# Gepetto/mpc-interface

Measured on AMD Instinct MI355X. Metric: QP assemblies/sec (P,q,G,h), biped N=16 batched, higher is better.
Workload: dtype f64; 1 GPU; C2 biped LIPM N=16 no=36 nc=76, per-instance (A,B)/given/aim, K1 on chip; batch_per_gpu=4096, global_batch=4096, streams=2

## Files before the change

include/mpcasm.h:

```cpp
#ifndef MPCASM_H
#define MPCASM_H

#include <stddef.h>
#include <stdint.h>

#ifdef __cplusplus
extern "C" {
#endif

typedef enum mpcasm_status {
  MPCASM_OK = 0,
  MPCASM_ERR_ARG = -1,
  MPCASM_ERR_PLAN = -2,
  MPCASM_ERR_HIP = -3,
  MPCASM_ERR_NODEVICE = -4,
  MPCASM_ERR_LIMIT = -5
} mpcasm_status;

typedef struct mpcasm_plan mpcasm_plan;


int mpcasm_abi_version(void);
int mpcasm_device_count(void);
int mpcasm_last_hip(void);
const char* mpcasm_status_string(int status);
enum { MPCASM_OPT_PATH = 1, MPCASM_OPT_PHASE_MASK = 2, MPCASM_OPT_RESIDENT_PER_CU = 3, MPCASM_OPT_JIT = 4,
       MPCASM_OPT_P_DIRECT = 5, MPCASM_OPT_RESIDENT_GRID = 6, MPCASM_OPT_JIT_FETCH_RUNS = 7 };
int mpcasm_set_option(int option, int value);
int mpcasm_plan_set_option(mpcasm_plan* plan, int option, int value);
int mpcasm_resident_lds_bytes(const int32_t* h_itab, size_t n_itab, const double* h_dtab, size_t n_dtab,
                              int64_t out[2]);
int mpcasm_jit_check(const int32_t* h_itab, size_t n_itab, const double* h_dtab, size_t n_dtab,
                     char* log, size_t log_capacity);
int mpcasm_fetch_segments(const int32_t* h_itab, size_t n_itab, const double* h_dtab, size_t n_dtab,
                          int limit, int32_t* out, size_t capacity, int64_t* n_words);

int mpcasm_plan_prepare(const mpcasm_plan* plan, int batch);
int mpcasm_jit_stats(int64_t out[3]);

int mpcasm_fill_su(const double* d_A, const double* d_B, double* d_S, double* d_U,
                   int batch, int N, int n, int m, int ltv, void* stream);

int mpcasm_plan_create(const int32_t* h_itab, size_t n_itab,
                       const double* h_dtab, size_t n_dtab,
                       mpcasm_plan** out_plan);
int mpcasm_plan_destroy(mpcasm_plan* plan);

int mpcasm_plan_sizes(const mpcasm_plan* plan, int64_t out[8]);

int mpcasm_plan_csc_sizes(const mpcasm_plan* plan, int64_t out[2]);
// ... 105 lines not shown
```

mpc-interface_amd/csrc/capi.hip:

```cpp
#include <hip/hip_runtime.h>
#include <stdint.h>
#include <stdlib.h>
#include <string.h>

#include <algorithm>
#include <cmath>
#include <mutex>
#include <new>
#include <string>
#include <vector>

#include "jit.h"
#include "kernels.h"

using namespace mpcasm;

namespace mpcasm {
int g_p_direct = 0;
extern int g_path;
extern int g_phase_mask;
extern int g_resident_per_cu, g_resident_grid;
}

struct mpcasm_plan {
// ... 1052 lines not shown
    g_phase_mask = value;
    return MPCASM_OK;
  }
  if (option == MPCASM_OPT_P_DIRECT) {
    if (value < 0 || value > 2) return MPCASM_ERR_ARG;
    g_p_direct = value;
    return MPCASM_OK;
  }
  if (option == MPCASM_OPT_JIT) {
    if (value < 0 || value > 2) return MPCASM_ERR_ARG;
    g_jit = value;
    return MPCASM_OK;
  }
  if (option == MPCASM_OPT_RESIDENT_PER_CU) {
    if (value < 0 || value > 16) return MPCASM_ERR_ARG;
    g_resident_per_cu = value;
    return MPCASM_OK;
  }
  if (option == MPCASM_OPT_JIT_FETCH_RUNS) {
    if (value < 0 || value > FS_MAX) return MPCASM_ERR_ARG;
    g_jit_fetch_runs = value;
    return MPCASM_OK;
  }
  if (option == MPCASM_OPT_RESIDENT_GRID) {
    if (value < 0 || value > (1 << 20)) return MPCASM_ERR_ARG;
    g_resident_grid = value;
    return MPCASM_OK;
  }
  return MPCASM_ERR_ARG;
}

int mpcasm_plan_set_option(mpcasm_plan* plan, int option, int value) {
  if (!plan) return MPCASM_ERR_ARG;
  if (option == MPCASM_OPT_PATH && value >= -1 && value <= 4) plan->opt_path = value;
  else if (option == MPCASM_OPT_JIT && value >= -1 && value <= 2) plan->opt_jit = value;
  else if (option == MPCASM_OPT_RESIDENT_PER_CU && value >= -1 && value <= 16) plan->opt_per_cu = value;
  else if (option == MPCASM_OPT_RESIDENT_GRID && value >= -1 && value <= (1 << 20)) plan->opt_grid = value;
  else return MPCASM_ERR_ARG;
  return MPCASM_OK;
}

const char* mpcasm_status_string(int status) {
  switch (status) {
    case MPCASM_OK: return "ok";
    case MPCASM_ERR_ARG: return "invalid argument";
    case MPCASM_ERR_PLAN: return "malformed plan tables";
// ... 76 lines not shown
  const int rc = validate_plan(h_itab, h_dtab, n_itab, n_dtab);
  if (rc != MPCASM_OK) return rc;
  PlanDev d;
  memset(&d, 0, sizeof d);
  plan_dev_from_tables(h_itab, &d);
  for (int direct = 0; direct < 2; ++direct) {
    d.rs_p_direct = 1 - direct;
    out[direct] = (int64_t)resident_lds_bytes(d);
  }
  return MPCASM_OK;
}

int mpcasm_jit_check(const int32_t* h_itab, size_t n_itab, const double* h_dtab, size_t n_dtab,
                     char* log, size_t log_capacity) {
  if (!h_itab || (n_dtab && !h_dtab)) return MPCASM_ERR_ARG;
  if (log && log_capacity) log[0] = 0;
  const int rc = validate_plan(h_itab, h_dtab, n_itab, n_dtab);
  if (rc != MPCASM_OK) return rc;
  PlanDev d;
  memset(&d, 0, sizeof d);
  plan_dev_from_tables(h_itab, &d);
  if (!d.rs_ok) return MPCASM_ERR_LIMIT;
  std::vector<char> code;
  std::string text;
  const int small = resident_p_direct_for(d, 1), large = resident_p_direct_for(d, 1 << 30);
  int out = MPCASM_OK;
  if (!jit_available()) {
    text = "libhiprtc.so could not be loaded";
    out = MPCASM_ERR_LIMIT;
  } else {
    for (int form : {small, large}) {
      if (form == large && small != large && out != MPCASM_OK) break;
      d.rs_p_direct = form;
      out = jit_code_for(jit_spec_header(d, h_itab, g_jit_fetch_runs), false, 0xBF, &code, &text) ? MPCASM_OK : MPCASM_ERR_HIP;
      if (small == large) break;
    }
  }
  if (log && log_capacity) {
    strncpy(log, text.c_str(), log_capacity - 1);
    log[log_capacity - 1] = 0;
  }
  return out;
}

int mpcasm_fetch_segments(const int32_t* h_itab, size_t n_itab, const double* h_dtab, size_t n_dtab,
                          int limit, int32_t* out, size_t capacity, int64_t* n_words) {
  if (!h_itab || (n_dtab && !h_dtab) || !n_words || (capacity && !out) || limit < 0) return MPCASM_ERR_ARG;
  const int rc = validate_plan(h_itab, h_dtab, n_itab, n_dtab);
  if (rc != MPCASM_OK) return rc;
  PlanDev d;
  memset(&d, 0, sizeof d);
  plan_dev_from_tables(h_itab, &d);
  if (!d.rs_ok) return MPCASM_ERR_LIMIT;
  const std::vector<int32_t> words = jit_fetch_plan(d, h_itab, limit);
  *n_words = (int64_t)words.size();
  if (words.size() > capacity) return MPCASM_ERR_LIMIT;
  if (!words.empty()) memcpy(out, words.data(), words.size() * sizeof(int32_t));
  return MPCASM_OK;
}
// ... 496 lines not shown
```

mpc-interface_amd/csrc/device_prims.h:

```cpp
#pragma once
#ifndef __HIPCC_RTC__
#include <hip/hip_runtime.h>
#include <stdint.h>
#endif

namespace mpcasm {

typedef double f64x4 __attribute__((ext_vector_type(4)));

__device__ __forceinline__ f64x4 mfma_f64_16x16x4(double a, double b, f64x4 c) {
  return __builtin_amdgcn_mfma_f64_16x16x4f64(a, b, c, 0, 0, 0);
}
__device__ __forceinline__ double mfma_f64_4x4x4(double a, double b, double c) {
  return __builtin_amdgcn_mfma_f64_4x4x4f64(a, b, c, 0, 0, 0);
}

template <int OA, int OB, int RB>
__device__ __forceinline__ double mfma_trip16(unsigned pa, unsigned pb, double sum) {
  static_assert(OA >= 0 && OB >= 0 && OA + 3 * RB < 65536 && OB + 3 * RB < 65536, "ds_read offset field");
  double a0, a1, a2, a3, b0, b1, b2, b3;
  asm volatile(
      "ds_read_b64 %1, %9 offset:%11\n\t"
      "ds_read_b64 %5, %10 offset:%15\n\t"
      "ds_read_b64 %2, %9 offset:%12\n\t"
      "ds_read_b64 %6, %10 offset:%16\n\t"
      "ds_read_b64 %3, %9 offset:%13\n\t"
      "ds_read_b64 %7, %10 offset:%17\n\t"
      "ds_read_b64 %4, %9 offset:%14\n\t"
      "ds_read_b64 %8, %10 offset:%18\n\t"
      "s_waitcnt lgkmcnt(6)\n\t"
      "v_mfma_f64_4x4x4_4b_f64 %0, %1, %5, %0\n\t"
      "s_waitcnt lgkmcnt(4)\n\t"
      "s_nop 2\n\t"
      "v_mfma_f64_4x4x4_4b_f64 %0, %2, %6, %0\n\t"
      "s_waitcnt lgkmcnt(2)\n\t"
      "s_nop 2\n\t"
      "v_mfma_f64_4x4x4_4b_f64 %0, %3, %7, %0\n\t"
      "s_waitcnt lgkmcnt(0)\n\t"
      "s_nop 2\n\t"
      "v_mfma_f64_4x4x4_4b_f64 %0, %4, %8, %0\n\t"
      "s_nop 5"
      : "+v"(sum), "=&v"(a0), "=&v"(a1), "=&v"(a2), "=&v"(a3), "=&v"(b0), "=&v"(b1), "=&v"(b2), "=&v"(b3)
      : "v"(pa), "v"(pb), "n"(OA), "n"(OA + RB), "n"(OA + 2 * RB), "n"(OA + 3 * RB), "n"(OB),
        "n"(OB + RB), "n"(OB + 2 * RB), "n"(OB + 3 * RB));
  return sum;
}

__device__ __forceinline__ double mfma_trip16_at(unsigned pa, unsigned pb, unsigned row_bytes, double sum) {
  double a0, a1, a2, a3, b0, b1, b2, b3;
  const unsigned pa1 = pa + row_bytes, pa2 = pa1 + row_bytes, pa3 = pa2 + row_bytes;
  const unsigned pb1 = pb + row_bytes, pb2 = pb1 + row_bytes, pb3 = pb2 + row_bytes;
  asm volatile(
      "ds_read_b64 %1, %9\n\t"
      "ds_read_b64 %5, %13\n\t"
      "ds_read_b64 %2, %10\n\t"
      "ds_read_b64 %6, %14\n\t"
      "ds_read_b64 %3, %11\n\t"
      "ds_read_b64 %7, %15\n\t"
      "ds_read_b64 %4, %12\n\t"
      "ds_read_b64 %8, %16\n\t"
      "s_waitcnt lgkmcnt(6)\n\t"
      "v_mfma_f64_4x4x4_4b_f64 %0, %1, %5, %0\n\t"
      "s_waitcnt lgkmcnt(4)\n\t"
      "s_nop 2\n\t"
      "v_mfma_f64_4x4x4_4b_f64 %0, %2, %6, %0\n\t"
      "s_waitcnt lgkmcnt(2)\n\t"
      "s_nop 2\n\t"
      "v_mfma_f64_4x4x4_4b_f64 %0, %3, %7, %0\n\t"
      "s_waitcnt lgkmcnt(0)\n\t"
// ... 41 lines not shown
```

mpc-interface_amd/csrc/jit.h:

```cpp
#pragma once
#include <hip/hip_runtime.h>
#include <stdint.h>

#include <string>
#include <vector>

#include "plan_dev.h"

namespace mpcasm {

extern int g_jit;
extern int g_jit_fetch_runs;
extern int g_phase_mask;

std::string jit_spec_header(const PlanDev& d, const int32_t* h_itab, int seg_limit = FS_MAX);
std::vector<int32_t> jit_fetch_plan(const PlanDev& d, const int32_t* h_itab, int seg_limit);
int jit_compile(const std::string& header, std::vector<char>* code, std::string* log,
                bool stamps = false, int phases = 0xBF);
const void* jit_kernel_for(const PlanDev& d, const int32_t* h_itab, int device, int batch,
                           size_t lds_bytes);
bool jit_code_for(const std::string& header, bool stamps, int phases, std::vector<char>* code,
                  std::string* log, bool distrust_disk = false);
bool jit_available();
void jit_stats(long out[3]);
void jit_forget(const void* itab);
int jit_launch(const void* kernel, const PlanDev& p, const SrcTable& src, const double* params,
               const double* given, double* P, double* q, double* G, double* h, int batch,
               int num_cus, int per_cu_limit, int grid_limit, void* work, hipStream_t stream, hipError_t* err);

}
```

mpc-interface_amd/csrc/jit.hip:

```cpp
#include <dlfcn.h>
#include <hip/hip_runtime.h>
#include <stdint.h>
#include <stdio.h>
#include <stdlib.h>
#include <string.h>

#include <sys/stat.h>
#include <sys/types.h>
#include <unistd.h>

#include <atomic>
#include <condition_variable>
#include <iterator>
#include <map>
#include <mutex>
#include <string>
#include <vector>

#include "jit.h"
#include "kernels.h"

namespace mpcasm {

int g_jit = 0;
int g_jit_fetch_runs = FS_MAX;

namespace {

#include "jit_embed.inc"

constexpr int JIT_MIN_BATCH = 512;

struct Rtc {
  typedef struct _hiprtcProgram* Program;
  int (*create)(Program*, const char*, const char*, int, const char* const*, const char* const*);
  int (*compile)(Program, int, const char* const*);
  int (*log_size)(Program, size_t*);
  int (*get_log)(Program, char*);
  int (*code_size)(Program, size_t*);
  int (*get_code)(Program, char*);
  int (*destroy)(Program*);
  bool ok = false;
};

const Rtc& rtc() {
  static Rtc r;
  static std::once_flag once;
  std::call_once(once, [] {
// ... 101 lines not shown
        for (int w = 0; w < FS_WORDS; ++w) append(table, w ? ", %lld" : "%lld", g < n ? fetch[at + 3 + g * FS_WORDS + w] : 0);
        table += "}, ";
      }
      table += "},\n";
    }
    if (chunks == 0) counts = "0", table = "  {},\n";
    s += std::string("constexpr int FSEG_") + name + "_N[] = {" + counts + "};\n";
    s += std::string("constexpr int FSEG_") + name + "[][8][6] = {\n" + table + "};\n";
    s += std::string("constexpr unsigned FSEG_") + name + "_TABLE = ";
    append(s, "%lldu;\n", on_table);
  }
  s += "constexpr int LTI[4][8] = {\n";
  for (int g = 0; g < RS_LTI_MAX; ++g) {
    s += "  {";
    for (int w = 0; w < RS_LTI_WORDS; ++w)
      append(s, w ? ", %lld" : "%lld", g < d.rs_nlti ? it[d.off_rs_lti + g * RS_LTI_WORDS + w] : 0);
    s += "},\n";
  }
  s += "};\n}  // namespace spec\n}  // namespace mpcasm\n";
  return s;
}

int jit_compile(const std::string& header, std::vector<char>* code, std::string* log, bool stamps,
                int phases) {
  const Rtc& r = rtc();
  if (!r.ok) {
    if (log) *log = "libhiprtc.so could not be loaded";
    return MPCASM_ERR_LIMIT;
  }
  const char* headers[] = {header.c_str(), k_src_device_prims, k_src_plan_dev, k_src_plan_tables};
  const char* names[] = {"plan_spec.h", "device_prims.h", "plan_dev.h", "plan_tables.h"};
  Rtc::Program prog = nullptr;
  if (r.create(&prog, k_src_resident, "resident.hip", 4, headers, names) != 0) return MPCASM_ERR_HIP;
  const char* waves = getenv("MPCASM_JIT_WAVES_PER_EU");
  const std::string wopt = std::string("-DMPCASM_SPEC_WAVES_PER_EU=") + (waves ? waves : "4");
  const char* last = stamps ? "-DMPCASM_SPEC_STAMPS=1"
                            : (getenv("MPCASM_JIT_PLAIN_STORES") ? "-DMPCASM_PLAIN_STORES=1" : "-DMPCASM_SPEC_NT=1");
  char popt[48];
  snprintf(popt, sizeof popt, "-DMPCASM_SPEC_PHASES=%d", phases);
  const char* opts[] = {"--offload-arch=gfx950", "-O3", "-std=c++17", "-DMPCASM_SPEC=1", wopt.c_str(), last, popt};
  const int rc = r.compile(prog, phases >= 0 ? 7 : 6, opts);
  size_t n = 0;
  if (log && r.log_size(prog, &n) == 0 && n > 1) {
    log->resize(n);
    r.get_log(prog, &(*log)[0]);
  }
  int out = MPCASM_ERR_HIP;
  if (rc == 0 && r.code_size(prog, &n) == 0 && n > 0) {
    code->resize(n);
    if (r.get_code(prog, code->data()) == 0) out = MPCASM_OK;
  }
  r.destroy(&prog);
  if (const char* dump = getenv("MPCASM_JIT_DUMP")) {
    const std::string base(dump);
    if (FILE* f = fopen((base + ".h").c_str(), "w")) {
      fwrite(header.data(), 1, header.size(), f);
      fclose(f);
    }
    if (out == MPCASM_OK)
      if (FILE* f = fopen((base + ".co").c_str(), "wb")) {
        fwrite(code->data(), 1, code->size(), f);
        fclose(f);
      }
  }
// ... 70 lines not shown
  if (!f) return;
  const bool ok = fwrite(code.data(), 1, code.size(), f) == code.size();
  fclose(f);
  if (ok && rename(tmp.c_str(), path.c_str()) == 0)
    ++g_stat_disk_writes;
  else
    (void)unlink(tmp.c_str());
}

struct JitKernel {
  hipModule_t module = nullptr;
  hipFunction_t fn = nullptr;
  int per_cu = 0;
  size_t lds = 0;
  bool failed = false;
  bool building = true;
};

std::mutex g_mutex;
std::condition_variable g_built;
std::map<std::pair<int, std::string>, JitKernel*> g_cache;
struct FastKey {
  const void* itab;
  int device, p_direct, phases, fetch_runs;
  bool operator<(const FastKey& o) const {
    if (fetch_runs != o.fetch_runs) return fetch_runs < o.fetch_runs;
    if (itab != o.itab) return itab < o.itab;
    if (device != o.device) return device < o.device;
    if (p_direct != o.p_direct) return p_direct < o.p_direct;
    return phases < o.phases;
  }
};
std::map<FastKey, JitKernel*> g_fast;

}

bool jit_code_for(const std::string& header, bool stamps, int phases, std::vector<char>* code,
                  std::string* log_out, bool distrust_disk) {
  const char* waves = getenv("MPCASM_JIT_WAVES_PER_EU");
  const std::string options = std::string(stamps ? "stamps " : "") + "phases " + std::to_string(phases) +
                              " waves " + (waves ? waves : "4") +
                              (getenv("MPCASM_JIT_PLAIN_STORES") ? " plain-stores" : "");
  const std::string dir = cache_dir();
  const std::string path = dir.empty() ? "" : dir + "/" + cache_key(header, options) + ".co";
  if (distrust_disk && !path.empty()) (void)unlink(path.c_str());
  if (!distrust_disk && !path.empty() && disk_read(path, code)) {
    ++g_stat_disk_hits;
    if (getenv("MPCASM_JIT_VERBOSE")) fprintf(stderr, "mpcasm: jit: code object from %s\n", path.c_str());
    return true;
  }
  std::string log;
  const int rc = jit_compile(header, code, &log, stamps, phases);
  if (log_out) *log_out = log;
  if (rc != MPCASM_OK) {
    if (getenv("MPCASM_JIT_VERBOSE")) fprintf(stderr, "mpcasm: jit failed:\n%s\n", log.c_str());
    return false;
  }
  ++g_stat_compiled;
  if (getenv("MPCASM_JIT_VERBOSE")) fprintf(stderr, "mpcasm: jit: compiled (%zu bytes)\n", code->size());
  if (!path.empty()) disk_write(path, *code);
  return true;
}

namespace {
}

const void* jit_kernel_for(const PlanDev& d, const int32_t* h_itab, int device, int batch,
                           size_t lds_bytes) {
  if (t_jit == 2) return nullptr;
  const bool stamps = (g_phase_mask & 64) != 0;
  const int phases = stamps ? -1 : g_phase_mask;
  const FastKey fast{d.itab, stamps ? device + 4096 : device, d.rs_p_direct, phases, g_jit_fetch_runs};
  const bool may_build = t_jit == 1 || batch >= JIT_MIN_BATCH;
  JitKernel* slot = nullptr;
  bool mine = false;
  std::string header;
  {
    std::unique_lock<std::mutex> lock(g_mutex);
    auto found = g_fast.find(fast);
    if (found != g_fast.end()) {
      slot = found->second;
    } else if (may_build) {
      header = jit_spec_header(d, h_itab, fast.fetch_runs);
      JitKernel*& by_text = g_cache[std::make_pair(fast.device, header + "//" + std::to_string(phases))];
      if (by_text == nullptr) {
        by_text = new JitKernel();
        mine = true;
      }
      slot = by_text;
      g_fast[fast] = slot;
    } else {
      return nullptr;
    }
    if (!mine) {
      if (slot->building && !may_build) return nullptr;
      g_built.wait(lock, [&] { return !slot->building; });
    }
  }
  if (mine) {
    std::vector<char> code;
    hipModule_t module = nullptr;
    hipFunction_t fn = nullptr;
    bool ok = false;
    for (int attempt = 0; attempt < 2 && !ok; ++attempt) {
      code.clear();
      const long hits = g_stat_disk_hits;
      ok = jit_code_for(header, stamps, phases, &code, nullptr, attempt == 1);
      const bool from_disk = g_stat_disk_hits != hits;
      if (ok && (hipModuleLoadData(&module, code.data()) != hipSuccess ||
                 hipModuleGetFunction(&fn, module, "resident_spec_kernel") != hipSuccess)) {
        (void)hipGetLastError();
        if (module) (void)hipModuleUnload(module);
        module = nullptr;
        fn = nullptr;
        ok = false;
        if (!from_disk) break;
      } else if (!ok) {
        break;
      }
    }
    if (ok && hipFuncSetAttribute(reinterpret_cast<const void*>(fn), hipFuncAttributeMaxDynamicSharedMemorySize,
                                  CU_LDS_BYTES) != hipSuccess) {
      (void)hipGetLastError();
      if (hipFuncSetAttribute(reinterpret_cast<const void*>(fn), hipFuncAttributeMaxDynamicSharedMemorySize,
                              RESIDENT_LDS_LIMIT) != hipSuccess) {
        (void)hipGetLastError();
        ok = false;
      }
    }
    {
// ... 61 lines not shown
```

mpc-interface_amd/csrc/resident.hip:

```cpp
#ifdef __HIPCC_RTC__
using __hip_internal::int32_t;
using __hip_internal::int64_t;
using __hip_internal::uint32_t;
using __hip_internal::uint64_t;
typedef unsigned long uintptr_t;
#else
#include <hip/hip_runtime.h>
#include <stdint.h>
#endif

#include "device_prims.h"
#include "plan_dev.h"
#ifdef MPCASM_SPEC
#include "plan_spec.h"
#endif
#ifndef __HIPCC_RTC__
#include "kernels.h"
#endif

namespace mpcasm {

#ifndef __HIPCC_RTC__
extern int g_phase_mask;
extern int g_resident_per_cu;
// ... 92 lines not shown
    case 3: asm volatile("s_waitcnt vmcnt(3)" ::: "memory"); break;
    case 4: asm volatile("s_waitcnt vmcnt(4)" ::: "memory"); break;
    default: asm volatile("s_waitcnt vmcnt(0)" ::: "memory"); break;
  }
}

__device__ __forceinline__ int resident_trip_row(int lk) { return ((lk & 1) << 3) | ((lk & 2) << 1); }

#ifdef MPCASM_SPEC
struct TripState {
  const char* Vlane;
  const char* prc;
  double *Pl, *ql;
  int ldpl;
  bool mirror;
  const double* dvec;
  int lx, lg, lk;
  const char *ap, *bp;
  int bi, bj;
  bool isq, live;
  double acc, sum;
};

template <int I>
__device__ __forceinline__ void spec_trip(TripState& s) {
  using PC = spec::PlanConst;
  constexpr int A = spec::TRIPS[I][RT_A], B = spec::TRIPS[I][RT_B], D = spec::TRIPS[I][RT_D];
  constexpr int W = spec::TRIPS[I][RT_W], AIM = spec::TRIPS[I][RT_AIM], WORD = spec::TRIPS[I][RT_WORD];
  constexpr int BI = spec::TRIPS[I][RT_BI], BJ = spec::TRIPS[I][RT_BJ];
  constexpr int row_bytes = PC::rs_ldv * 8, ldp = (PC::no + 1) & ~1;
  constexpr int qmask = (WORD >> RT_QMASK) & 15, livemask = (WORD >> RT_LIVE) & 15;
  constexpr bool nop = (WORD >> RT_NOP) & 1, half = (WORD >> RT_HALF) & 1;
  if constexpr ((WORD >> RT_FIRST) & 1) {
    int lg_ = s.lg;
    asm volatile("" : "+v"(lg_));
    s.bi = (BI >> (8 * lg_)) & 255;
    s.bj = (BJ >> (8 * lg_)) & 255;
    s.isq = (qmask >> lg_) & 1;
    s.live = (livemask >> lg_) & 1;
    s.ap = s.Vlane + s.bi * 32;
    s.bp = s.Vlane + (s.isq ? 0 : s.bj * 32);
    s.acc = 0.0;
  }
  if constexpr ((WORD & 31) != 0) {
    const char* bsrc = qmask == 0 ? s.bp + B : (qmask == livemask ? s.bp + D : s.bp + (s.isq ? D : B));
    if constexpr (!((WORD >> RT_SHORT) & 1)) {
      constexpr int span = 3 * row_bytes;
      constexpr int AH = A + span < 65536 ? 0 : A, DH = D + span < 65536 ? 0 : D, BH = B + span < 65536 ? 0 : B;
      const unsigned pa = (unsigned)(uintptr_t)s.ap + AH;
      if constexpr (qmask == 0) {
        s.sum = mfma_trip16<A - AH, B - BH, row_bytes>(pa, (unsigned)(uintptr_t)s.bp + BH, s.sum);
      } else if constexpr (qmask == livemask) {
        s.sum = mfma_trip16<A - AH, D - DH, row_bytes>(pa, (unsigned)(uintptr_t)s.bp + DH, s.sum);
      } else {
        s.sum = mfma_trip16<A - AH, B - BH, row_bytes>(pa, (unsigned)(uintptr_t)s.bp + BH + (s.isq ? D - B : 0), s.sum);
      }
    } else {
      const int short_shift = (s.lk - resident_trip_row(s.lk)) * row_bytes;
      const double a = *reinterpret_cast<const double*>(s.ap + (A + short_shift));
      const double b = *reinterpret_cast<const double*>(bsrc + short_shift);
      s.sum = mfma_f64_4x4x4(a, b, s.sum);
    }
    if constexpr ((WORD >> RT_TERM_END) & 1) {
      const double w = *reinterpret_cast<const double*>(s.prc + W);
      if constexpr (qmask != 0 || nop) {
        const double aim = *reinterpret_cast<const double*>(s.prc + AIM);
        const double ws = half ? 0.5 * w : w;
        const double ones = quad_broadcast<1>(s.sum);
        const double m = s.isq ? ws : (nop ? 0.0 : w);
        s.acc = fma(m, fma(-(s.isq ? aim : 0.0), ones, s.sum), s.acc);
      } else {
        s.acc = fma(w, s.sum, s.acc);
      }
      s.sum = 0.0;
    }
  }
  if constexpr ((WORD >> RT_LAST) & 1) {
    int lk_ = s.lk, lx_ = s.lx;
    asm volatile("" : "+v"(lk_), "+v"(lx_));
    const int row = 4 * s.bi + lk_, col = 4 * s.bj + lx_;
    if (s.live && row < PC::no) {
      if (s.isq) {
        if (lx_ == 0) s.ql[row] = s.acc + s.dvec[ldp + row];
      } else if (col < PC::no) {
        const double val = s.acc + (row == col ? s.dvec[col] : 0.0);
        s.Pl[row * s.ldpl + col] = val;
        if (PC::rs_sym && s.bi != s.bj) s.Pl[col * s.ldpl + row] = val;
      }
    }
  }
}

struct LaneSrc {
  const char* base;
  long long stride;
  bool isg;
  int2 entry;
};
static_assert(FS_MAX == 8 && FS_WORDS == 6 && RS_LTI_MAX == 4 && RS_LTI_WORDS == 8, "plan_spec.h, as jit.hip writes it");
template <bool AB, int K>
constexpr int spec_fetch_runs() {
  if constexpr (AB)
    return K < spec::PlanConst::rs_ab / 32 ? spec::FSEG_AB_N[K] : 0;
  else
    return K < spec::PlanConst::rs_nchunk ? spec::FSEG_IMG_N[K] : 0;
}
template <bool AB, int K, int S>
__device__ __forceinline__ void spec_lane_run(LaneSrc& out, int lane, const SrcTable& src, const double* params,
                                              const double* given, const double* plan_dtab) {
  using PC = spec::PlanConst;
  if constexpr (S < spec_fetch_runs<AB, K>()) {
    constexpr int first = AB ? spec::FSEG_AB[K][S][FS_FIRST] : spec::FSEG_IMG[K][S][FS_FIRST];
    constexpr int lanes = AB ? spec::FSEG_AB[K][S][FS_LANES] : spec::FSEG_IMG[K][S][FS_LANES];
// ... 57 lines not shown
}
template <int K>
__device__ __forceinline__ void spec_first_image(int lane, long inst, long ginst, unsigned img_lds, const SrcTable& src,
                                                 const double* params, const double* given, const double* plan_dtab) {
  using PC = spec::PlanConst;
  if constexpr (K < PC::rs_nchunk && K < 32) {
    if constexpr (spec_fetch_runs<false, K>() != 0) {
      const LaneSrc m = spec_lane_src<false, K>(lane, src, params, given, plan_dtab);
      const char* a = m.base + (m.isg ? ginst : inst) * m.stride;
      if constexpr (PC::rs_unit == 16)
        dma16(a, img_lds + (unsigned)(K * 64 * 16));
      else
        dma4(a, img_lds + (unsigned)(K * 64 * 4));
    }
    spec_first_image<K + 1>(lane, inst, ginst, img_lds, src, params, given, plan_dtab);
  }
}
constexpr bool spec_ab_by_runs() {
  for (int k = 0; k < spec::PlanConst::rs_ab / 32; ++k)
    if (spec::FSEG_AB_N[k] == 0) return false;
  return true;
}

template <int I, int N>
__device__ __forceinline__ void spec_trips(TripState& s) {
  if constexpr (I < N) {
    spec_trip<I>(s);
    __builtin_amdgcn_sched_barrier(0);
    spec_trips<I + 1, N>(s);
  }
}
template <int WAVE>
__device__ __forceinline__ void spec_wave_trips(TripState& s) {
  spec_trips<spec::WTRIP[WAVE][0], spec::WTRIP[WAVE][0] + spec::WTRIP[WAVE][1]>(s);
}
#endif

template <int JC, bool STAMPS, bool GEN, class PlanT>
__device__ __forceinline__ void resident_body(
    const PlanT& p, const int32_t* __restrict__ plan_itab, const double* __restrict__ plan_dtab,
    const SrcTable& src, const double* __restrict__ params, const double* __restrict__ given,
    double* __restrict__ P, double* __restrict__ q, double* __restrict__ G,
    double* __restrict__ h, int batch, int phases, unsigned long long* __restrict__ stamps) {
  extern __shared__ __attribute__((aligned(16))) double lds[];
  const int tid = threadIdx.x, lane = tid & 63;
  const int wave = __builtin_amdgcn_readfirstlane(tid >> 6);
  unsigned long long t_acc[8] = {0, 0, 0, 0, 0, 0, 0, 0}, t_prev = 0;
  const unsigned long long t_begin = STAMPS ? __builtin_amdgcn_s_memtime() : 0;
#define SETUP_STAMP(k)                                                                  \
  if (STAMPS && stamps != nullptr && lane == 0)                                         \
    stamps[((size_t)gridDim.x + blockIdx.x) * (NT / 64) * 8 + wave * 8 + (k)] =         \
        __builtin_amdgcn_s_memtime() - t_begin;
  const bool stamping = STAMPS && stamps != nullptr;
#define MPCASM_STAMP(slot)                                         \
  if (STAMPS && stamping) {                                        \
    const unsigned long long t_now = __builtin_amdgcn_s_memtime(); \
    t_acc[slot] += t_now - t_prev;                                 \
// ... 1053 lines not shown
```

mpc-interface_amd/mpcasm/capi.py:

```python
import ctypes
import os

_HERE = os.path.dirname(os.path.abspath(__file__))
LIB_PATH = os.environ.get("MPCASM_LIB") or os.path.join(_HERE, "libmpcasm.so")

OK = 0
ERR_LIMIT = -5
OPT_PATH = 1
OPT_PHASE_MASK = 2
OPT_RESIDENT_PER_CU = 3
OPT_RESIDENT_GRID = 6
OPT_P_DIRECT = 5
OPT_JIT_FETCH_RUNS = 7
OPT_JIT = 4
PHASE_DEFAULT = 0xBF
PHASE_STAMPS = 0x40
STATUS = {
    0: "MPCASM_OK",
    -1: "MPCASM_ERR_ARG",
    -2: "MPCASM_ERR_PLAN",
    -3: "MPCASM_ERR_HIP",
    -4: "MPCASM_ERR_NODEVICE",
    -5: "MPCASM_ERR_LIMIT",
}
QP_SOLVED, QP_MAX_ITER, QP_PRIMAL_INFEASIBLE, QP_DUAL_INFEASIBLE, QP_NON_CVX = 1, -2, -3, -4, -7
QP_STATUS = {
    1: "MPCASM_QP_SOLVED",
    -2: "MPCASM_QP_MAX_ITER",
    -3: "MPCASM_QP_PRIMAL_INFEASIBLE",
    -4: "MPCASM_QP_DUAL_INFEASIBLE",
    -7: "MPCASM_QP_NON_CVX",
}
GIVEN_KEEP, GIVEN_CONST = -1, -2


def qp_bit(status):
# ... 131 lines not shown
```

Before: 176.9 million assemblies/s.

## Software-pipeline LDS operand reads across JIT trips with depth autotuned by spills

```diff
diff --git a/include/mpcasm.h b/include/mpcasm.h
--- a/include/mpcasm.h
+++ b/include/mpcasm.h
@@ -25,7 +25,8 @@
 int mpcasm_last_hip(void);
 const char* mpcasm_status_string(int status);
 enum { MPCASM_OPT_PATH = 1, MPCASM_OPT_PHASE_MASK = 2, MPCASM_OPT_RESIDENT_PER_CU = 3, MPCASM_OPT_JIT = 4,
-       MPCASM_OPT_P_DIRECT = 5, MPCASM_OPT_RESIDENT_GRID = 6, MPCASM_OPT_JIT_FETCH_RUNS = 7 };
+       MPCASM_OPT_P_DIRECT = 5, MPCASM_OPT_RESIDENT_GRID = 6, MPCASM_OPT_JIT_FETCH_RUNS = 7,
+       MPCASM_OPT_JIT_TRIP_DEPTH = 8 };
 int mpcasm_set_option(int option, int value);
 int mpcasm_plan_set_option(mpcasm_plan* plan, int option, int value);
 int mpcasm_resident_lds_bytes(const int32_t* h_itab, size_t n_itab, const double* h_dtab, size_t n_dtab,
diff --git a/mpc-interface_amd/csrc/capi.hip b/mpc-interface_amd/csrc/capi.hip
--- a/mpc-interface_amd/csrc/capi.hip
+++ b/mpc-interface_amd/csrc/capi.hip
@@ -1098,6 +1098,11 @@
     g_jit_fetch_runs = value;
     return MPCASM_OK;
   }
+  if (option == MPCASM_OPT_JIT_TRIP_DEPTH) {
+    if (value < -1 || value > 2) return MPCASM_ERR_ARG;
+    g_jit_trip_depth = value;
+    return MPCASM_OK;
+  }
   if (option == MPCASM_OPT_RESIDENT_GRID) {
     if (value < 0 || value > (1 << 20)) return MPCASM_ERR_ARG;
     g_resident_grid = value;
@@ -1220,7 +1225,7 @@
   plan_dev_from_tables(h_itab, &d);
   if (!d.rs_ok) return MPCASM_ERR_LIMIT;
   std::vector<char> code;
-  std::string text;
+  std::string text, choices;
   const int small = resident_p_direct_for(d, 1), large = resident_p_direct_for(d, 1 << 30);
   int out = MPCASM_OK;
   if (!jit_available()) {
@@ -1230,9 +1235,13 @@
     for (int form : {small, large}) {
       if (form == large && small != large && out != MPCASM_OK) break;
       d.rs_p_direct = form;
-      out = jit_code_for(jit_spec_header(d, h_itab, g_jit_fetch_runs), false, 0xBF, &code, &text) ? MPCASM_OK : MPCASM_ERR_HIP;
+      std::string choice;
+      out = jit_code_for(jit_spec_header(d, h_itab, g_jit_fetch_runs), false, 0xBF, &code, &text, false,
+                         g_jit_trip_depth, &choice) ? MPCASM_OK : MPCASM_ERR_HIP;
+      if (!choice.empty()) choices += std::string("P ") + (form ? "direct" : "in LDS") + ": " + choice + "\n";
       if (small == large) break;
     }
+    text = choices + text;
   }
   if (log && log_capacity) {
     strncpy(log, text.c_str(), log_capacity - 1);
diff --git a/mpc-interface_amd/csrc/device_prims.h b/mpc-interface_amd/csrc/device_prims.h
--- a/mpc-interface_amd/csrc/device_prims.h
+++ b/mpc-interface_amd/csrc/device_prims.h
@@ -45,6 +45,95 @@
         "n"(OB + RB), "n"(OB + 2 * RB), "n"(OB + 3 * RB));
   return sum;
 }
+
+struct TripOps {
+  double a0, a1, a2, a3, b0, b1, b2, b3;
+};
+template <int OA, int OB, int RB>
+__device__ __forceinline__ void trip16_ask(unsigned pa, unsigned pb, TripOps& o) {
+  static_assert(OA >= 0 && OB >= 0 && OA + 3 * RB < 65536 && OB + 3 * RB < 65536, "ds_read offset field");
+  asm volatile(
+      "ds_read_b64 %0, %8 offset:%10\n\t"
+      "ds_read_b64 %4, %9 offset:%14\n\t"
+      "ds_read_b64 %1, %8 offset:%11\n\t"
+      "ds_read_b64 %5, %9 offset:%15\n\t"
+      "ds_read_b64 %2, %8 offset:%12\n\t"
+      "ds_read_b64 %6, %9 offset:%16\n\t"
+      "ds_read_b64 %3, %8 offset:%13\n\t"
+      "ds_read_b64 %7, %9 offset:%17"
+      : "=&v"(o.a0), "=&v"(o.a1), "=&v"(o.a2), "=&v"(o.a3), "=&v"(o.b0), "=&v"(o.b1), "=&v"(o.b2), "=&v"(o.b3)
+      : "v"(pa), "v"(pb), "n"(OA), "n"(OA + RB), "n"(OA + 2 * RB), "n"(OA + 3 * RB), "n"(OB), "n"(OB + RB),
+        "n"(OB + 2 * RB), "n"(OB + 3 * RB));
+}
+template <int O, int RB>
+__device__ __forceinline__ void trip16_ask4(unsigned p, double& r0, double& r1, double& r2, double& r3) {
+  static_assert(O >= 0 && O + 3 * RB < 65536, "ds_read offset field");
+  asm volatile(
+      "ds_read_b64 %0, %4 offset:%5\n\t"
+      "ds_read_b64 %1, %4 offset:%6\n\t"
+      "ds_read_b64 %2, %4 offset:%7\n\t"
+      "ds_read_b64 %3, %4 offset:%8"
+      : "=&v"(r0), "=&v"(r1), "=&v"(r2), "=&v"(r3)
+      : "v"(p), "n"(O), "n"(O + RB), "n"(O + 2 * RB), "n"(O + 3 * RB));
+}
+template <int O>
+__device__ __forceinline__ void lds_ask(unsigned p, double& r) {
+  static_assert(O >= 0 && O < 65536, "ds_read offset field");
+  asm volatile("ds_read_b64 %0, %1 offset:%2" : "=&v"(r) : "v"(p), "n"(O));
+}
+#define MPCASM_TRIP16_MUL_TEXT                                  \
+  "s_waitcnt lgkmcnt(%[n0])\n\t"                                \
+  "s_nop 0\n\t"                                                 \
+  "v_mfma_f64_4x4x4_4b_f64 %[sum], %[a0], %[b0], %[sum]\n\t"    \
+  "s_waitcnt lgkmcnt(%[n1])\n\t"                                \
+  "s_nop 2\n\t"                                                 \
+  "v_mfma_f64_4x4x4_4b_f64 %[sum], %[a1], %[b1], %[sum]\n\t"    \
+  "s_waitcnt lgkmcnt(%[n2])\n\t"                                \
+  "s_nop 2\n\t"                                                 \
+  "v_mfma_f64_4x4x4_4b_f64 %[sum], %[a2], %[b2], %[sum]\n\t"    \
+  "s_waitcnt lgkmcnt(%[n3])\n\t"                                \
+  "s_nop 2\n\t"                                                 \
+  "v_mfma_f64_4x4x4_4b_f64 %[sum], %[a3], %[b3], %[sum]\n\t"    \
+  "s_nop 5"
+#define MPCASM_TRIP_MUL_TERM "\n\ts_waitcnt lgkmcnt(%[nend])"
+#define MPCASM_TRIP16_MUL_IN                                                                                        \
+  [a0] "v"(o.a0), [a1] "v"(o.a1), [a2] "v"(o.a2), [a3] "v"(o.a3), [b0] "v"(o.b0), [b1] "v"(o.b1), [b2] "v"(o.b2), \
+      [b3] "v"(o.b3), [n0] "n"(N0), [n1] "n"(N1), [n2] "n"(N2), [n3] "n"(N3), [nend] "n"(N3 - NP)
+template <int N0, int N1, int N2, int N3, int NP>
+__device__ __forceinline__ double trip16_mul(const TripOps& o, double sum, double& w, double& aim) {
+  static_assert(N0 >= 0 && N1 >= 0 && N2 >= 0 && N3 >= 0 && N0 <= 15 && N1 <= 15 && N2 <= 15 && N3 <= 15,
+                "lgkmcnt field");
+  static_assert(NP >= 0 && NP <= 2 && N3 >= NP, "the term's reads are behind the operands");
+  if constexpr (NP == 2)
+    asm volatile(MPCASM_TRIP16_MUL_TEXT MPCASM_TRIP_MUL_TERM : [sum] "+v"(sum), "+v"(w), "+v"(aim) : MPCASM_TRIP16_MUL_IN);
+  else if constexpr (NP == 1)
+    asm volatile(MPCASM_TRIP16_MUL_TEXT MPCASM_TRIP_MUL_TERM : [sum] "+v"(sum), "+v"(w) : MPCASM_TRIP16_MUL_IN);
+  else
+    asm volatile(MPCASM_TRIP16_MUL_TEXT : [sum] "+v"(sum) : MPCASM_TRIP16_MUL_IN);
+  return sum;
+}
+#undef MPCASM_TRIP16_MUL_TEXT
+#undef MPCASM_TRIP16_MUL_IN
+#define MPCASM_TRIP4_MUL_TEXT \
+  "s_waitcnt lgkmcnt(%[n])\n\ts_nop 0\n\tv_mfma_f64_4x4x4_4b_f64 %[sum], %[a], %[b], %[sum]\n\ts_nop 5"
+template <int N, int NP>
+__device__ __forceinline__ double trip4_mul(double a, double b, double sum, double& w, double& aim) {
+  static_assert(N >= 0 && N <= 15, "lgkmcnt field");
+  static_assert(NP >= 0 && NP <= 2 && N >= NP, "the term's reads are behind the operands");
+  if constexpr (NP == 2)
+    asm volatile(MPCASM_TRIP4_MUL_TEXT MPCASM_TRIP_MUL_TERM
+                 : [sum] "+v"(sum), "+v"(w), "+v"(aim)
+                 : [a] "v"(a), [b] "v"(b), [n] "n"(N), [nend] "n"(N - NP));
+  else if constexpr (NP == 1)
+    asm volatile(MPCASM_TRIP4_MUL_TEXT MPCASM_TRIP_MUL_TERM
+                 : [sum] "+v"(sum), "+v"(w)
+                 : [a] "v"(a), [b] "v"(b), [n] "n"(N), [nend] "n"(N - NP));
+  else
+    asm volatile(MPCASM_TRIP4_MUL_TEXT : [sum] "+v"(sum) : [a] "v"(a), [b] "v"(b), [n] "n"(N));
+  return sum;
+}
+#undef MPCASM_TRIP4_MUL_TEXT
+#undef MPCASM_TRIP_MUL_TERM
 
 __device__ __forceinline__ double mfma_trip16_at(unsigned pa, unsigned pb, unsigned row_bytes, double sum) {
   double a0, a1, a2, a3, b0, b1, b2, b3;
diff --git a/mpc-interface_amd/csrc/jit.h b/mpc-interface_amd/csrc/jit.h
--- a/mpc-interface_amd/csrc/jit.h
+++ b/mpc-interface_amd/csrc/jit.h
@@ -11,16 +11,22 @@
 
 extern int g_jit;
 extern int g_jit_fetch_runs;
+extern int g_jit_trip_depth;
 extern int g_phase_mask;
 
 std::string jit_spec_header(const PlanDev& d, const int32_t* h_itab, int seg_limit = FS_MAX);
 std::vector<int32_t> jit_fetch_plan(const PlanDev& d, const int32_t* h_itab, int seg_limit);
 int jit_compile(const std::string& header, std::vector<char>* code, std::string* log,
-                bool stamps = false, int phases = 0xBF);
+                bool stamps = false, int phases = 0xBF, int depth = 0);
+struct JitFigures {
+  int vgprs = 0, vgpr_spill = 0, scratch = 0;
+};
+bool jit_code_figures(const std::vector<char>& code, JitFigures* out);
 const void* jit_kernel_for(const PlanDev& d, const int32_t* h_itab, int device, int batch,
                            size_t lds_bytes);
 bool jit_code_for(const std::string& header, bool stamps, int phases, std::vector<char>* code,
-                  std::string* log, bool distrust_disk = false);
+                  std::string* log, bool distrust_disk = false, int trip_depth = -1,
+                  std::string* choice = nullptr);
 bool jit_available();
 void jit_stats(long out[3]);
 void jit_forget(const void* itab);
diff --git a/mpc-interface_amd/csrc/jit.hip b/mpc-interface_amd/csrc/jit.hip
--- a/mpc-interface_amd/csrc/jit.hip
+++ b/mpc-interface_amd/csrc/jit.hip
@@ -24,6 +24,7 @@
 
 int g_jit = 0;
 int g_jit_fetch_runs = FS_MAX;
+int g_jit_trip_depth = -1;
 
 namespace {
 
@@ -171,7 +172,7 @@
 }
 
 int jit_compile(const std::string& header, std::vector<char>* code, std::string* log, bool stamps,
-                int phases) {
+                int phases, int depth) {
   const Rtc& r = rtc();
   if (!r.ok) {
     if (log) *log = "libhiprtc.so could not be loaded";
@@ -187,8 +188,12 @@
                             : (getenv("MPCASM_JIT_PLAIN_STORES") ? "-DMPCASM_PLAIN_STORES=1" : "-DMPCASM_SPEC_NT=1");
   char popt[48];
   snprintf(popt, sizeof popt, "-DMPCASM_SPEC_PHASES=%d", phases);
-  const char* opts[] = {"--offload-arch=gfx950", "-O3", "-std=c++17", "-DMPCASM_SPEC=1", wopt.c_str(), last, popt};
-  const int rc = r.compile(prog, phases >= 0 ? 7 : 6, opts);
+  char dopt[48];
+  snprintf(dopt, sizeof dopt, "-DMPCASM_SPEC_TRIP_DEPTH=%d", depth);
+  std::vector<const char*> opts = {"--offload-arch=gfx950", "-O3", "-std=c++17", "-DMPCASM_SPEC=1", wopt.c_str(), last};
+  if (phases >= 0) opts.push_back(popt);
+  if (depth > 0) opts.push_back(dopt);
+  const int rc = r.compile(prog, (int)opts.size(), opts.data());
   size_t n = 0;
   if (log && r.log_size(prog, &n) == 0 && n > 1) {
     log->resize(n);
@@ -305,9 +310,10 @@
 std::map<std::pair<int, std::string>, JitKernel*> g_cache;
 struct FastKey {
   const void* itab;
-  int device, p_direct, phases, fetch_runs;
+  int device, p_direct, phases, fetch_runs, trip_depth;
   bool operator<(const FastKey& o) const {
     if (fetch_runs != o.fetch_runs) return fetch_runs < o.fetch_runs;
+    if (trip_depth != o.trip_depth) return trip_depth < o.trip_depth;
     if (itab != o.itab) return itab < o.itab;
     if (device != o.device) return device < o.device;
     if (p_direct != o.p_direct) return p_direct < o.p_direct;
@@ -318,29 +324,130 @@
 
 }
 
+bool jit_code_figures(const std::vector<char>& code, JitFigures* out) {
+  auto figure = [&](const char* key, int* value) {
+    const size_t n = strlen(key);
+    bool found = false;
+    *value = 0;
+    for (size_t at = 0; at + n + 1 <= code.size(); ++at) {
+      if (memcmp(code.data() + at, key, n) != 0) continue;
+      const unsigned char* v = reinterpret_cast<const unsigned char*>(code.data()) + at + n;
+      const size_t left = code.size() - at - n;
+      long long x = -1;
+      if (v[0] < 0x80) x = v[0];
+      else if (v[0] == 0xcc && left >= 2) x = v[1];
+      else if (v[0] == 0xcd && left >= 3) x = (v[1] << 8) | v[2];
+      else if (v[0] == 0xce && left >= 5) x = ((long long)v[1] << 24) | (v[2] << 16) | (v[3] << 8) | v[4];
+      if (x < 0) continue;
+      found = true;
+      if (x > *value) *value = (int)x;
+    }
+    return found;
+  };
+  JitFigures f;
+  if (!figure(".vgpr_count", &f.vgprs) || !figure(".vgpr_spill_count", &f.vgpr_spill) ||
+      !figure(".private_segment_fixed_size", &f.scratch))
+    return false;
+  *out = f;
+  return true;
+}
+
+namespace {
+
+std::string figures_text(int depth, bool known, const JitFigures& f) {
+  char buf[128];
+  if (known)
+    snprintf(buf, sizeof buf, "depth %d: %d VGPRs, %d spilled, scratch %d", depth, f.vgprs, f.vgpr_spill, f.scratch);
+  else
+    snprintf(buf, sizeof buf, "depth %d: no figures", depth);
+  return buf;
+}
+
+}
+
 bool jit_code_for(const std::string& header, bool stamps, int phases, std::vector<char>* code,
-                  std::string* log_out, bool distrust_disk) {
+                  std::string* log_out, bool distrust_disk, int trip_depth, std::string* choice_out) {
   const char* waves = getenv("MPCASM_JIT_WAVES_PER_EU");
   const std::string options = std::string(stamps ? "stamps " : "") + "phases " + std::to_string(phases) +
                               " waves " + (waves ? waves : "4") +
                               (getenv("MPCASM_JIT_PLAIN_STORES") ? " plain-stores" : "");
+  const bool forced = trip_depth >= 0;
   const std::string dir = cache_dir();
-  const std::string path = dir.empty() ? "" : dir + "/" + cache_key(header, options) + ".co";
-  if (distrust_disk && !path.empty()) (void)unlink(path.c_str());
-  if (!distrust_disk && !path.empty() && disk_read(path, code)) {
-    ++g_stat_disk_hits;
-    if (getenv("MPCASM_JIT_VERBOSE")) fprintf(stderr, "mpcasm: jit: code object from %s\n", path.c_str());
+  auto path_of = [&](int depth) {
+    const std::string o = options + (forced ? " trip-depth forced " + std::to_string(depth)
+                                            : (depth ? " trip-depth " + std::to_string(depth) : ""));
+    return dir.empty() ? std::string() : dir + "/" + cache_key(header, o) + ".co";
+  };
+  const bool verbose = getenv("MPCASM_JIT_VERBOSE") != nullptr;
+  std::string choice;
+  for (int depth = forced ? trip_depth : 2; depth >= (forced ? trip_depth : 0); --depth) {
+    const std::string path = path_of(depth);
+    if (path.empty()) break;
+    if (distrust_disk) {
+      (void)unlink(path.c_str());
+    } else if (disk_read(path, code)) {
+      ++g_stat_disk_hits;
+      if (verbose) fprintf(stderr, "mpcasm: jit: code object from %s (trip depth %d)\n", path.c_str(), depth);
+      JitFigures f;
+      const bool known = jit_code_figures(*code, &f);
+      if (choice_out)
+        *choice_out = "trip depth " + std::to_string(depth) + (forced ? " (forced)" : " (automatic)") +
+                      ", from the disk cache; " + figures_text(depth, known, f);
+      return true;
+    }
+  }
+  std::string log;
+  auto compile = [&](int depth, std::vector<char>* out, JitFigures* f, bool* known) {
+    std::string one;
+    const int rc = jit_compile(header, out, &one, stamps, phases, depth);
+    log += one;
+    if (rc != MPCASM_OK) {
+      if (verbose) fprintf(stderr, "mpcasm: jit failed (trip depth %d):\n%s\n", depth, one.c_str());
+      return false;
+    }
+    ++g_stat_compiled;
+    *known = jit_code_figures(*out, f);
+    if (verbose)
+      fprintf(stderr, "mpcasm: jit: compiled (%zu bytes; %s)\n", out->size(), figures_text(depth, *known, *f).c_str());
+    choice += (choice.empty() ? "" : "; ") + figures_text(depth, *known, *f);
     return true;
-  }
-  std::string log;
-  const int rc = jit_compile(header, code, &log, stamps, phases);
+  };
+  int chosen = -1;
+  JitFigures f{};
+  bool known = false;
+  if (forced) {
+    if (compile(trip_depth, code, &f, &known)) chosen = trip_depth;
+  } else {
+    std::vector<char> base;
+    JitFigures f0{};
+    bool known0 = false, have0 = false;
+    for (int depth = 2; depth >= 1 && chosen < 0; --depth) {
+      std::vector<char> deep;
+      if (!compile(depth, &deep, &f, &known) || !known || f.vgpr_spill != 0) continue;
+      if (f.scratch != 0) {
+        if (!have0) {
+          have0 = true;
+          if (!compile(0, &base, &f0, &known0)) break;
+        }
+        if (!known0 || f.scratch > f0.scratch) continue;
+      }
+      chosen = depth;
+      code->swap(deep);
+    }
+    if (chosen < 0) {
+      if (!have0 && compile(0, &base, &f0, &known0)) have0 = true;
+      if (have0 && !base.empty()) {
+        chosen = 0;
+        code->swap(base);
+      }
+    }
+  }
   if (log_out) *log_out = log;
-  if (rc != MPCASM_OK) {
-    if (getenv("MPCASM_JIT_VERBOSE")) fprintf(stderr, "mpcasm: jit failed:\n%s\n", log.c_str());
-    return false;
-  }
-  ++g_stat_compiled;
-  if (getenv("MPCASM_JIT_VERBOSE")) fprintf(stderr, "mpcasm: jit: compiled (%zu bytes)\n", code->size());
+  if (chosen < 0) return false;
+  choice = "trip depth " + std::to_string(chosen) + (forced ? " (forced); " : " (automatic: the deepest without spilled VGPRs and with no more scratch than depth 0); ") + choice;
+  if (verbose) fprintf(stderr, "mpcasm: jit: %s\n", choice.c_str());
+  if (choice_out) *choice_out = choice;
+  const std::string path = path_of(chosen);
   if (!path.empty()) disk_write(path, *code);
   return true;
 }
@@ -353,7 +460,7 @@
   if (t_jit == 2) return nullptr;
   const bool stamps = (g_phase_mask & 64) != 0;
   const int phases = stamps ? -1 : g_phase_mask;
-  const FastKey fast{d.itab, stamps ? device + 4096 : device, d.rs_p_direct, phases, g_jit_fetch_runs};
+  const FastKey fast{d.itab, stamps ? device + 4096 : device, d.rs_p_direct, phases, g_jit_fetch_runs, g_jit_trip_depth};
   const bool may_build = t_jit == 1 || batch >= JIT_MIN_BATCH;
   JitKernel* slot = nullptr;
   bool mine = false;
@@ -365,7 +472,7 @@
       slot = found->second;
     } else if (may_build) {
       header = jit_spec_header(d, h_itab, fast.fetch_runs);
-      JitKernel*& by_text = g_cache[std::make_pair(fast.device, header + "//" + std::to_string(phases))];
+      JitKernel*& by_text = g_cache[std::make_pair(fast.device, header + "//" + std::to_string(phases) + "/" + std::to_string(fast.trip_depth))];
       if (by_text == nullptr) {
         by_text = new JitKernel();
         mine = true;
@@ -388,7 +495,7 @@
     for (int attempt = 0; attempt < 2 && !ok; ++attempt) {
       code.clear();
       const long hits = g_stat_disk_hits;
-      ok = jit_code_for(header, stamps, phases, &code, nullptr, attempt == 1);
+      ok = jit_code_for(header, stamps, phases, &code, nullptr, attempt == 1, fast.trip_depth);
       const bool from_disk = g_stat_disk_hits != hits;
       if (ok && (hipModuleLoadData(&module, code.data()) != hipSuccess ||
                  hipModuleGetFunction(&fn, module, "resident_spec_kernel") != hipSuccess)) {
diff --git a/mpc-interface_amd/csrc/resident.hip b/mpc-interface_amd/csrc/resident.hip
--- a/mpc-interface_amd/csrc/resident.hip
+++ b/mpc-interface_amd/csrc/resident.hip
@@ -138,60 +138,102 @@
   double acc, sum;
 };
 
+struct PackLane {
+  const char *ap, *bp;
+  int bi, bj;
+  bool isq, live;
+};
 template <int I>
-__device__ __forceinline__ void spec_trip(TripState& s) {
+__device__ __forceinline__ PackLane spec_pack_lane(const TripState& s) {
+  constexpr int WORD = spec::TRIPS[I][RT_WORD], BI = spec::TRIPS[I][RT_BI], BJ = spec::TRIPS[I][RT_BJ];
+  constexpr int qmask = (WORD >> RT_QMASK) & 15, livemask = (WORD >> RT_LIVE) & 15;
+  PackLane k;
+  int lg_ = s.lg;
+  asm volatile("" : "+v"(lg_));
+  k.bi = (BI >> (8 * lg_)) & 255;
+  k.bj = (BJ >> (8 * lg_)) & 255;
+  k.isq = (qmask >> lg_) & 1;
+  k.live = (livemask >> lg_) & 1;
+  k.ap = s.Vlane + k.bi * 32;
+  k.bp = s.Vlane + (k.isq ? 0 : k.bj * 32);
+  return k;
+}
+template <int I>
+__device__ __forceinline__ void spec_pack_first(TripState& s) {
+  if constexpr ((spec::TRIPS[I][RT_WORD] >> RT_FIRST) & 1) {
+    const PackLane k = spec_pack_lane<I>(s);
+    s.bi = k.bi;
+    s.bj = k.bj;
+    s.isq = k.isq;
+    s.live = k.live;
+    s.ap = k.ap;
+    s.bp = k.bp;
+    s.acc = 0.0;
+  }
+}
+template <int I>
+struct TripAddr {
+  static constexpr int A = spec::TRIPS[I][RT_A], B = spec::TRIPS[I][RT_B], D = spec::TRIPS[I][RT_D];
+  static constexpr int WORD = spec::TRIPS[I][RT_WORD];
+  static constexpr int qmask = (WORD >> RT_QMASK) & 15, livemask = (WORD >> RT_LIVE) & 15;
+  static constexpr int row_bytes = spec::PlanConst::rs_ldv * 8, span = 3 * row_bytes;
+  static constexpr int AH = A + span < 65536 ? 0 : A, DH = D + span < 65536 ? 0 : D, BH = B + span < 65536 ? 0 : B;
+  static constexpr int OA = A - AH;
+  static constexpr int OB = qmask != 0 && qmask == livemask ? D - DH : B - BH;
+  static __device__ __forceinline__ unsigned pa(const char* ap) { return (unsigned)(uintptr_t)ap + AH; }
+  static __device__ __forceinline__ unsigned pb(const char* bp, bool isq) {
+    if constexpr (qmask == 0) {
+      return (unsigned)(uintptr_t)bp + BH;
+    } else if constexpr (qmask == livemask) {
+      return (unsigned)(uintptr_t)bp + DH;
+    } else {
+      return (unsigned)(uintptr_t)bp + BH + (isq ? D - B : 0);
+    }
+  }
+};
+template <int I>
+__device__ __forceinline__ void spec_trip_short(TripState& s) {
+  constexpr int A = spec::TRIPS[I][RT_A], B = spec::TRIPS[I][RT_B], D = spec::TRIPS[I][RT_D];
+  constexpr int WORD = spec::TRIPS[I][RT_WORD], row_bytes = spec::PlanConst::rs_ldv * 8;
+  constexpr int qmask = (WORD >> RT_QMASK) & 15, livemask = (WORD >> RT_LIVE) & 15;
+  const char* bsrc = qmask == 0 ? s.bp + B : (qmask == livemask ? s.bp + D : s.bp + (s.isq ? D : B));
+  const int short_shift = (s.lk - resident_trip_row(s.lk)) * row_bytes;
+  const double a = *reinterpret_cast<const double*>(s.ap + (A + short_shift));
+  const double b = *reinterpret_cast<const double*>(bsrc + short_shift);
+  s.sum = mfma_f64_4x4x4(a, b, s.sum);
+}
+template <int I>
+constexpr bool spec_term_aim() {
+  return ((spec::TRIPS[I][RT_WORD] >> RT_QMASK) & 15) != 0 || ((spec::TRIPS[I][RT_WORD] >> RT_NOP) & 1);
+}
+template <int I>
+__device__ __forceinline__ void spec_term_end(TripState& s, double w, double aim) {
+  constexpr int WORD = spec::TRIPS[I][RT_WORD];
+  constexpr bool nop = (WORD >> RT_NOP) & 1, half = (WORD >> RT_HALF) & 1;
+  if constexpr (spec_term_aim<I>()) {
+    const double ws = half ? 0.5 * w : w;
+    const double ones = quad_broadcast<1>(s.sum);
+    const double m = s.isq ? ws : (nop ? 0.0 : w);
+    s.acc = fma(m, fma(-(s.isq ? aim : 0.0), ones, s.sum), s.acc);
+  } else {
+    s.acc = fma(w, s.sum, s.acc);
+  }
+  s.sum = 0.0;
+}
+template <int I>
+__device__ __forceinline__ void spec_term_end(TripState& s) {
+  if constexpr ((spec::TRIPS[I][RT_WORD] >> RT_TERM_END) & 1) {
+    const double w = *reinterpret_cast<const double*>(s.prc + spec::TRIPS[I][RT_W]);
+    double aim = 0.0;
+    if constexpr (spec_term_aim<I>()) aim = *reinterpret_cast<const double*>(s.prc + spec::TRIPS[I][RT_AIM]);
+    spec_term_end<I>(s, w, aim);
+  }
+}
+template <int I>
+__device__ __forceinline__ void spec_pack_last(TripState& s) {
   using PC = spec::PlanConst;
-  constexpr int A = spec::TRIPS[I][RT_A], B = spec::TRIPS[I][RT_B], D = spec::TRIPS[I][RT_D];
-  constexpr int W = spec::TRIPS[I][RT_W], AIM = spec::TRIPS[I][RT_AIM], WORD = spec::TRIPS[I][RT_WORD];
-  constexpr int BI = spec::TRIPS[I][RT_BI], BJ = spec::TRIPS[I][RT_BJ];
-  constexpr int row_bytes = PC::rs_ldv * 8, ldp = (PC::no + 1) & ~1;
-  constexpr int qmask = (WORD >> RT_QMASK) & 15, livemask = (WORD >> RT_LIVE) & 15;
-  constexpr bool nop = (WORD >> RT_NOP) & 1, half = (WORD >> RT_HALF) & 1;
-  if constexpr ((WORD >> RT_FIRST) & 1) {
-    int lg_ = s.lg;
-    asm volatile("" : "+v"(lg_));
-    s.bi = (BI >> (8 * lg_)) & 255;
-    s.bj = (BJ >> (8 * lg_)) & 255;
-    s.isq = (qmask >> lg_) & 1;
-    s.live = (livemask >> lg_) & 1;
-    s.ap = s.Vlane + s.bi * 32;
-    s.bp = s.Vlane + (s.isq ? 0 : s.bj * 32);
-    s.acc = 0.0;
-  }
-  if constexpr ((WORD & 31) != 0) {
-    const char* bsrc = qmask == 0 ? s.bp + B : (qmask == livemask ? s.bp + D : s.bp + (s.isq ? D : B));
-    if constexpr (!((WORD >> RT_SHORT) & 1)) {
-      constexpr int span = 3 * row_bytes;
-      constexpr int AH = A + span < 65536 ? 0 : A, DH = D + span < 65536 ? 0 : D, BH = B + span < 65536 ? 0 : B;
-      const unsigned pa = (unsigned)(uintptr_t)s.ap + AH;
-      if constexpr (qmask == 0) {
-        s.sum = mfma_trip16<A - AH, B - BH, row_bytes>(pa, (unsigned)(uintptr_t)s.bp + BH, s.sum);
-      } else if constexpr (qmask == livemask) {
-        s.sum = mfma_trip16<A - AH, D - DH, row_bytes>(pa, (unsigned)(uintptr_t)s.bp + DH, s.sum);
-      } else {
-        s.sum = mfma_trip16<A - AH, B - BH, row_bytes>(pa, (unsigned)(uintptr_t)s.bp + BH + (s.isq ? D - B : 0), s.sum);
-      }
-    } else {
-      const int short_shift = (s.lk - resident_trip_row(s.lk)) * row_bytes;
-      const double a = *reinterpret_cast<const double*>(s.ap + (A + short_shift));
-      const double b = *reinterpret_cast<const double*>(bsrc + short_shift);
-      s.sum = mfma_f64_4x4x4(a, b, s.sum);
-    }
-    if constexpr ((WORD >> RT_TERM_END) & 1) {
-      const double w = *reinterpret_cast<const double*>(s.prc + W);
-      if constexpr (qmask != 0 || nop) {
-        const double aim = *reinterpret_cast<const double*>(s.prc + AIM);
-        const double ws = half ? 0.5 * w : w;
-        const double ones = quad_broadcast<1>(s.sum);
-        const double m = s.isq ? ws : (nop ? 0.0 : w);
-        s.acc = fma(m, fma(-(s.isq ? aim : 0.0), ones, s.sum), s.acc);
-      } else {
-        s.acc = fma(w, s.sum, s.acc);
-      }
-      s.sum = 0.0;
-    }
-  }
-  if constexpr ((WORD >> RT_LAST) & 1) {
+  constexpr int ldp = (PC::no + 1) & ~1;
+  if constexpr ((spec::TRIPS[I][RT_WORD] >> RT_LAST) & 1) {
     int lk_ = s.lk, lx_ = s.lx;
     asm volatile("" : "+v"(lk_), "+v"(lx_));
     const int row = 4 * s.bi + lk_, col = 4 * s.bj + lx_;
@@ -205,6 +247,103 @@
       }
     }
   }
+}
+
+template <int I>
+__device__ __forceinline__ void spec_trip(TripState& s) {
+  constexpr int WORD = spec::TRIPS[I][RT_WORD];
+  spec_pack_first<I>(s);
+  if constexpr ((WORD & 31) != 0) {
+    if constexpr (!((WORD >> RT_SHORT) & 1)) {
+      using T = TripAddr<I>;
+      s.sum = mfma_trip16<T::OA, T::OB, T::row_bytes>(T::pa(s.ap), T::pb(s.bp, s.isq), s.sum);
+    } else {
+      spec_trip_short<I>(s);
+    }
+    spec_term_end<I>(s);
+  }
+  spec_pack_last<I>(s);
+}
+
+template <int I>
+constexpr int spec_trip_kind() {
+  return (spec::TRIPS[I][RT_WORD] & 31) == 0 ? 0 : ((spec::TRIPS[I][RT_WORD] >> RT_SHORT) & 1 ? 1 : 2);
+}
+template <int I, int WHAT>
+__device__ __forceinline__ void spec_ask(const TripState& s, const char* ap, const char* bp, bool isq, TripOps& o) {
+  using T = TripAddr<I>;
+  if constexpr (spec_trip_kind<I>() == 2) {
+    if constexpr (WHAT == 2)
+      trip16_ask<T::OA, T::OB, T::row_bytes>(T::pa(ap), T::pb(bp, isq), o);
+    else if constexpr (WHAT == 0)
+      trip16_ask4<T::OA, T::row_bytes>(T::pa(ap), o.a0, o.a1, o.a2, o.a3);
+    else
+      trip16_ask4<T::OB, T::row_bytes>(T::pb(bp, isq), o.b0, o.b1, o.b2, o.b3);
+  } else {
+    const unsigned short_shift = (unsigned)((s.lk - resident_trip_row(s.lk)) * T::row_bytes);
+    if constexpr (WHAT != 1) lds_ask<T::OA>(T::pa(ap) + short_shift, o.a0);
+    if constexpr (WHAT != 0) lds_ask<T::OB>(T::pb(bp, isq) + short_shift, o.b0);
+  }
+}
+template <int I, int DEPTH>
+constexpr int spec_asked_ahead() {
+  return spec_trip_kind<I>() == 2 ? (DEPTH >= 2 ? 8 : 4) : (spec_trip_kind<I>() == 1 ? (DEPTH >= 2 ? 2 : 1) : 0);
+}
+template <int I, int N, int DEPTH>
+__device__ __forceinline__ void spec_ask_next(TripState& s, TripOps& nxt) {
+  if constexpr (I + 1 < N) {
+    if constexpr (spec_trip_kind<I + 1>() != 0) {
+      const char *ap = s.ap, *bp = s.bp;
+      bool isq = s.isq;
+      if constexpr ((spec::TRIPS[I + 1][RT_WORD] >> RT_FIRST) & 1) {
+        const PackLane k = spec_pack_lane<I + 1>(s);
+        ap = k.ap, bp = k.bp, isq = k.isq;
+      }
+      spec_ask<I + 1, DEPTH >= 2 ? 2 : 0>(s, ap, bp, isq, nxt);
+    }
+  }
+}
+template <int I, int N, int DEPTH>
+constexpr int spec_asked_next() {
+  if constexpr (I + 1 < N) return spec_asked_ahead<I + 1, DEPTH>();
+  return 0;
+}
+constexpr int spec_lgkm(int n) { return n < 15 ? n : 15; }
+template <int I, int N, int I0, int DEPTH>
+__device__ __forceinline__ void spec_trip_piped(TripState& s, TripOps& cur, TripOps& nxt) {
+  constexpr int WORD = spec::TRIPS[I][RT_WORD], kind = spec_trip_kind<I>();
+  spec_pack_first<I>(s);
+  if constexpr (kind != 0) {
+    constexpr bool asked = I > I0;
+    constexpr bool term = (WORD >> RT_TERM_END) & 1, aims = term && spec_term_aim<I>();
+    if constexpr (!asked)
+      spec_ask<I, 2>(s, s.ap, s.bp, s.isq, cur);
+    else if constexpr (DEPTH < 2)
+      spec_ask<I, 1>(s, s.ap, s.bp, s.isq, cur);
+    double w = 0.0, aim = 0.0;
+    if constexpr (term) {
+      constexpr int W = spec::TRIPS[I][RT_W], WH = W < 65536 ? 0 : W;
+      lds_ask<W - WH>((unsigned)(uintptr_t)s.prc + WH, w);
+    }
+    if constexpr (aims) {
+      constexpr int AIM = spec::TRIPS[I][RT_AIM], MH = AIM < 65536 ? 0 : AIM;
+      lds_ask<AIM - MH>((unsigned)(uintptr_t)s.prc + MH, aim);
+    }
+    spec_ask_next<I, N, DEPTH>(s, nxt);
+    constexpr int np = (term ? 1 : 0) + (aims ? 1 : 0);
+    constexpr int later = np + spec_asked_next<I, N, DEPTH>();
+    if constexpr (kind == 2) {
+      constexpr int each = !asked || DEPTH >= 2 ? 2 : 1;
+      s.sum = trip16_mul<spec_lgkm(3 * each + later), spec_lgkm(2 * each + later), spec_lgkm(each + later),
+                         spec_lgkm(later), np>(cur, s.sum, w, aim);
+    } else {
+      s.sum = trip4_mul<spec_lgkm(later), np>(cur.a0, cur.b0, s.sum, w, aim);
+    }
+    if constexpr (term) spec_term_end<I>(s, w, aim);
+  } else {
+    spec_ask_next<I, N, DEPTH>(s, nxt);
+  }
+  spec_pack_last<I>(s);
 }
 
 struct LaneSrc {
@@ -308,6 +447,9 @@
   return true;
 }
 
+#ifndef MPCASM_SPEC_TRIP_DEPTH
+#define MPCASM_SPEC_TRIP_DEPTH 0
+#endif
 template <int I, int N>
 __device__ __forceinline__ void spec_trips(TripState& s) {
   if constexpr (I < N) {
@@ -316,9 +458,23 @@
     spec_trips<I + 1, N>(s);
   }
 }
+template <int I, int N, int I0, int DEPTH>
+__device__ __forceinline__ void spec_trips_piped(TripState& s, TripOps& cur, TripOps& nxt) {
+  if constexpr (I < N) {
+    spec_trip_piped<I, N, I0, DEPTH>(s, cur, nxt);
+    __builtin_amdgcn_sched_barrier(0);
+    spec_trips_piped<I + 1, N, I0, DEPTH>(s, nxt, cur);
+  }
+}
 template <int WAVE>
 __device__ __forceinline__ void spec_wave_trips(TripState& s) {
-  spec_trips<spec::WTRIP[WAVE][0], spec::WTRIP[WAVE][0] + spec::WTRIP[WAVE][1]>(s);
+  constexpr int I0 = spec::WTRIP[WAVE][0], N = spec::WTRIP[WAVE][0] + spec::WTRIP[WAVE][1];
+#if MPCASM_SPEC_TRIP_DEPTH == 0
+  spec_trips<I0, N>(s);
+#else
+  TripOps even, odd;
+  spec_trips_piped<I0, N, I0, MPCASM_SPEC_TRIP_DEPTH>(s, even, odd);
+#endif
 }
 #endif
 
diff --git a/mpc-interface_amd/mpcasm/capi.py b/mpc-interface_amd/mpcasm/capi.py
--- a/mpc-interface_amd/mpcasm/capi.py
+++ b/mpc-interface_amd/mpcasm/capi.py
@@ -12,6 +12,7 @@
 OPT_RESIDENT_GRID = 6
 OPT_P_DIRECT = 5
 OPT_JIT_FETCH_RUNS = 7
+OPT_JIT_TRIP_DEPTH = 8
 OPT_JIT = 4
 PHASE_DEFAULT = 0xBF
 PHASE_STAMPS = 0x40
```

New measurement: 172.2 million assemblies/s. -2.7%, worse.
